# RobotLocomotion/pytorch-dense-correspondence

Measured on AMD Instinct MI355X. Metric: training images/sec, 640x480 D=3 ResNet34-8s, higher is better.
Workload: dtype f32 (f16x3 products)

## Files before the change

include/dcn_hip.h:

```cpp
#ifndef DCN_HIP_H
#define DCN_HIP_H

#include <stddef.h>
#include <stdint.h>

#ifdef __cplusplus
extern "C" {
#endif

#define DCN_OK 0
#define DCN_E_INVALID (-1)
#define DCN_E_LAUNCH (-2)
#define DCN_E_UNSUPPORTED (-3)

const char* dcn_version(void);

void dcn_reload_env(void);

void dcn_release_pooled_buffers(void);


enum { DCN_LIST_MATCH = 0, DCN_LIST_MASKED = 1, DCN_LIST_BACKGROUND = 2, DCN_LIST_BLIND = 3, DCN_NUM_LISTS = 4 };

enum {
// ... 185 lines not shown
size_t dcn_conv_gemm_workspace_hl(const dcn_conv_desc* c, int dgrad);
int dcn_conv_hl_shape_info(const dcn_conv_desc* c, int dgrad, int* info6);
int dcn_split_act_hl32(const float* src, const float* absmax, void* dst, int64_t rows, int channels, void* stream);
int dcn_split_weights_hl32(int n, const float* const* w, void* const* out, const int* cout, const int* taps, const int* cin,
                           const int* ldn, int transposed, float scale, void* stream);
int dcn_conv_forward_hl(const dcn_conv_desc* c, const void* in_hl, const float* in_absmax, const void* w_hl, float w_scale,
                        const float* bias, float* out, float* bn_partial, void* workspace, void* stream);
int dcn_conv_dgrad_hl(const dcn_conv_desc* c, const void* dout_hl, const void* wt_hl, float w_scale, const float* dout_absmax,
                      const float* add, float* din, void* workspace, void* stream);

int dcn_conv_wgrad_hl_eligible(const dcn_conv_desc* c);
int dcn_conv_wgrad_hl_kind(const dcn_conv_desc* c);
size_t dcn_conv_wgrad_workspace_hl(const dcn_conv_desc* c);
int dcn_conv_wgrad_hl(const dcn_conv_desc* c, const void* x_hl, const float* x_absmax, const void* dout_hl,
                      const float* dout_absmax, float* dw, void* slabs, void* stream);

int dcn_split_stem_weights_f16(const float* w4, void* hi, void* lo, int cout, float scale, void* stream);
int dcn_conv_stem_forward_f16(const dcn_conv_desc* c, const float* in, const float* in_absmax, const void* w_hi, const void* w_lo,
                              float w_scale, float* out, float* bn_partial, void* stream);

int dcn_split_weights_f16(int n, const float* const* w, void* const* hi, void* const* lo, const int* cout, const int* taps,
                          const int* cin, const int* ldn, int transposed, float scale, void* stream);

int dcn_split_weights_scaled_f16(int n, const float* const* w, const float* const* row_scale, void* const* hi,
                                 void* const* lo, const int* cout, const int* taps, const int* cin, const int* ldn,
                                 int transposed, float scale, void* stream);
int dcn_conv_forward_fused_f16(const dcn_conv_desc* c, const float* in, const float* in_absmax, const void* w_hi,
                               const void* w_lo, float w_scale, const float* bias, const float* add, int relu, float* out,
                               float* out_absmax, void* workspace, void* stream);

// ... 263 lines not shown
```

pytorch-dense-correspondence_amd/csrc/backbone_engine.hip:

```cpp
#include <algorithm>
#include <cstdio>
#include <cstdlib>
#include <cstring>
#include <mutex>
#include <string>
#include <vector>

#include "dcn_tuning.h"
#include "elementwise_kernels.h"

namespace {

using dcn::ceil_div;

struct ConvL {
    double flops = 0;
    dcn_conv_desc d;
    int w = -1, b = -1;
    int bn = -1;
    size_t x = 0;
    int cin_true = 0;
    size_t wsplit = 0;
    size_t whl = 0;
    bool hl_any = false;
// ... 16 lines not shown
    size_t in = 0, mid[2] = {0, 0}, out = 0;
    int64_t out_rows = 0;
    int out_c = 0, in_c = 0;
    int64_t in_rows = 0;
    int act_in = -1, act_mid[2] = {-1, -1}, act_out = -1;
    int act_down = -1;
    size_t hl_mid[2] = {0, 0}, hl_in = 0;
    bool has_hl_mid[2] = {false, false}, has_hl_in = false;
};
struct ParamInfo {
    std::string name;
    int64_t shape[4];
    int ndim;
};

enum class Kernel : unsigned char { FP32, F16, HL, STEM8 };
struct ConvRoute { Kernel fwd, dgrad, wgrad; };

}

struct dcn_plan {
    std::string arch, prefix;
    int N = 0, H = 0, W = 0, D = 0, Dp = 0, base = 64;
    int groups = 1;
    bool bottleneck = false;
    std::vector<ConvL> convs;
    std::vector<BnL> bns;
    std::vector<BlockL> blocks;
    std::vector<ParamInfo> params;
    std::vector<std::pair<size_t, size_t>> relu_masks;
    int stem = -1, fc = -1;
// ... 34 lines not shown

namespace {

size_t align64(size_t x) { return (x + 63) & ~size_t(63); }

std::vector<ConvRoute> conv_routes(const dcn_plan& p, int conv_mode, bool reserving = false) {
    std::vector<ConvRoute> rt(p.convs.size(), ConvRoute{Kernel::FP32, Kernel::FP32, Kernel::FP32});
    if (conv_mode != DCN_CONV_F16X3) return rt;
    const dcn::Tuning& tune = dcn::tuning();
    for (const ConvL& c : p.convs) {
        ConvRoute& r = rt[c.idx];
        r.fwd = c.hl_any && dcn_conv_hl_eligible(&c.d, 0) != 0 ? Kernel::HL : Kernel::F16;
        r.dgrad = c.hl_any && dcn_conv_hl_eligible(&c.d, 1) != 0 ? Kernel::HL : Kernel::F16;
        const bool hl_x = reserving ? (c.idx != p.stem && c.idx != p.fc) : c.has_hl_x;
        r.wgrad = hl_x && dcn_conv_wgrad_hl_eligible(&c.d) != 0 ? Kernel::HL : Kernel::F16;
    }
    const dcn_conv_desc& sd = p.convs[p.stem].d;
    if (tune.stem8 != 0 && tune.gemm_uni != 0 && sd.win >= 8 && sd.kh == 7 && sd.cin == 4 && (int64_t)sd.n * sd.hin * sd.win * 16 <= ((int64_t)1 << 31))
        rt[p.stem].fwd = Kernel::STEM8;
    return rt;
}

struct Builder {
    dcn_plan& p;
    size_t saved = 0;
    explicit Builder(dcn_plan& pl) : p(pl) {}

    size_t alloc_saved(size_t floats) {
        const size_t o = saved;
        saved = align64(saved + floats);
// ... 910 lines not shown
    auto RT = [&](hipError_t e) { if (e != hipSuccess) rt_fail = 1; };
    if (overlap) {
        hipStreamCaptureStatus cs = hipStreamCaptureStatusNone;
        if (hipStreamIsCapturing(st, &cs) != hipSuccess || cs != hipStreamCaptureStatusNone) overlap = false;
    }
    int n_bn = 0, cur = 0;
    bool wg_pending[2] = {false, false};
    float* const dqbuf[2] = {R.Wk(p.w_dq), R.Wk(p.w_dq2)};
    float* const hlimg[2] = {R.hlbuf(0), R.hlbuf(1)};
    const float* dq_of = nullptr;
    const bool fuse_red = f16 && dcn::tuning().bn_bwd_fused != 0;
    p.fused_bn_bwd = 0;
    const float* red_dy = nullptr;
    int red_tiles = 0;
    const float* hl_dx_of = nullptr;
    auto bn_bwd = [&](const ConvL& c, const float* dy, const float* relu_out, float* dx, float* g_out, const float* dy2 = nullptr) {
        const BnL& b = p.bns[c.bn];
        const float* s = R.S(b.stats);
        const unsigned char* mask = relu_out ? R.M((size_t)(relu_out - R.saved)) : nullptr;
        cur = overlap ? (n_bn & 1) : 0;
        if (overlap && wg_pending[cur]) RT(hipStreamWaitEvent(st, p.ev_wg[cur], 0));
        const int tiles = (red_dy == dy && dy) ? red_tiles : 0;
        red_dy = nullptr;
        if (tiles > 0) { relu_out = nullptr; mask = nullptr; g_out = nullptr; ++p.fused_bn_bwd; }
        const bool prod = f16 && dcn::tuning().hl_producers != 0;
        const bool hl_d = prod && !fuse_red && routes[c.idx].dgrad == Kernel::HL;
        const bool hl_w = prod && routes[c.idx].wgrad == Kernel::HL;
        hl_dx_of = (hl_d || hl_w) ? dx : nullptr;
        dcn::launch_bn_bwd(dy, relu_out, mask, R.S(c.x), s, R.P(b.g), b.C, b.rows, p.groups, part, grads[b.g],
                           grads[b.b], k123, dx, g_out, f16 ? amax + c.idx : nullptr,
                           (f16 && !hl_w) ? (void*)dqbuf[cur] : nullptr, st, tiles, dy2,
                           (hl_d || hl_w) ? (void*)hlimg[cur] : nullptr, hl_d ? 0 : 1,
                           (overlap && dcn::tuning().bn_bwd_lean != 0) ? dcn::tuning().bn_bwd_lean_mask : 0);
        if (overlap) RT(hipEventRecord(p.ev_dq[cur], st));
        ++n_bn;
        dq_of = (f16 && !hl_w) ? dx : nullptr;
    };
    auto wgrad_launch = [&](const ConvL& c, auto&& launch) -> int {
        if (!overlap) return R.timed(1, c.flops, [&] { return launch(st); });
        RT(hipStreamWaitEvent(p.side, p.ev_dq[cur], 0));
        DCN_TRY(launch(p.side));
        RT(hipEventRecord(p.ev_wg[cur], p.side));
        wg_pending[cur] = true;
        return DCN_OK;
    };
    auto wgrad = [&](const ConvL& c, const float* in, const float* dx, float* dw) -> int {
        const Kernel k = routes[c.idx].wgrad;
        if (k == Kernel::FP32) return R.timed(1, c.flops, [&] { return dcn_conv_wgrad(&c.d, in, dx, dw, slab, st); });
        if (k == Kernel::HL) {
            const float* ximg = R.S(c.hl_x);
            if (hl_dx_of != dx) {
                DCN_TRY(R.other([&] { return dcn_split_act_hl32(dx, amax + c.idx, hlimg[cur], (int64_t)c.d.n * c.d.hout * c.d.wout, c.d.ldc, st); }));
                if (overlap) RT(hipEventRecord(p.ev_dq[cur], st));
                hl_dx_of = dx;
            }
            return wgrad_launch(c, [&](hipStream_t s) {
                return dcn_conv_wgrad_hl(&c.d, ximg, R.A(c.in_act), hlimg[cur], amax + c.idx, dw, slab, s);
            });
        }
        if (dq_of != dx) {
            DCN_TRY(R.other([&] { return dcn_split_grad_blocked_f16(dx, c.d.n * c.d.hout * c.d.wout, c.d.ldc, amax + c.idx, dqbuf[0], st); }));
            return R.timed(1, c.flops, [&] {
                return dcn_conv_wgrad_f16(&c.d, in, 1, R.A(c.in_act), dqbuf[0], amax + c.idx, dw, slab, st);
            });
        }
        return wgrad_launch(c, [&](hipStream_t s) {
            return dcn_conv_wgrad_f16(&c.d, in, 1, R.A(c.in_act), dqbuf[cur], amax + c.idx, dw, slab, s);
        });
    };
    auto dgrad = [&](const ConvL& c, const float* dx, const float* add, float* din, const ConvL* bn_of = nullptr,
                     const float* relu_out = nullptr) -> int {
        const ConvRoute& r = routes[c.idx];
        if (r.dgrad == Kernel::FP32) {
            DCN_TRY(R.other([&] { return dcn_transpose_weight(R.P(c.w), wt, c.d.cout, c.d.kh * c.d.kw, c.d.cin, c.d.ldc, st); }));
            return R.timed(0, c.flops, [&] { return dcn_conv_dgrad(&c.d, dx, wt, add, din, R.SK(c, 1, Kernel::FP32), st); });
        }
        if (fuse_red && bn_of) {
            const BnL& b = p.bns[bn_of->bn];
            const int tiles = dcn_conv_dgrad_bn_num_mtiles_f16(&c.d);
            if (tiles > 0 && tiles % p.groups == 0 && b.C == c.d.cin && b.rows == (int64_t)c.d.n * c.d.hin * c.d.win) {
                const unsigned char* mask = relu_out ? R.M((size_t)(relu_out - R.saved)) : nullptr;
                red_dy = din;
                red_tiles = tiles / p.groups;
// ... 107 lines not shown
        float* t = dout; dout = dnext; dnext = t;
        for (size_t k = 0; k + 1 < p.bucket_block.size(); ++k)
            if (p.bucket_block[k] == bi && p.bucket_state == 1) {
                if (overlap) {
                    RT(hipEventRecord(p.ev_bucket_side, p.side));
                    RT(hipStreamWaitEvent(st, p.ev_bucket_side, 0));
                }
                RT(hipEventRecord(p.ev_bucket[k], st));
            }
    }
    const ConvL& stem = p.convs[p.stem];
    const BnL& sb = p.bns[stem.bn];
    const int hp = (stem.d.hout + 2 - 3) / 2 + 1, wp = (stem.d.wout + 2 - 3) / 2 + 1;
    dcn::launch_maxpool_bwd(dout, (const unsigned char*)R.S(p.s_argmax), dnext, N, stem.d.hout, stem.d.wout, hp, wp, sb.C,
                            st, dout_add);
    bn_bwd(stem, dnext, R.S(p.s_stem_y), dxa, nullptr);
    DCN_TRY(wgrad(stem, R.S(p.s_in4), dxa, R.Wk(p.w_dwstem)));
    if (overlap) {
        RT(hipEventRecord(p.ev_join, p.side));
        RT(hipStreamWaitEvent(st, p.ev_join, 0));
    }
    dcn::launch_unpad_c4_to_c3(R.Wk(p.w_dwstem), grads[stem.w], (int64_t)p.base * 49, st);
    if (p.bucket_state == 1) RT(hipEventRecord(p.ev_bucket.back(), st));
    if (rt_fail) return DCN_E_LAUNCH;
    return dcn::check_launch();
}

}

extern "C" int dcn_backbone_backward(dcn_plan* plan, const float* grad_descriptors, const float* const* params,
                                     const void* saved, void* workspace, float* const* grads, int normalize,
// ... 10 lines not shown
```

pytorch-dense-correspondence_amd/csrc/conv_f16_kernels.hip:

```cpp
#include <algorithm>
#include <atomic>

#include "conv_shared.h"
#include "dcn_tuning.h"
#include "f16_split.h"

namespace {

using namespace dcnconv;
using namespace dcnsplit;

constexpr int HBK = 32;
constexpr int LDH = HBK + 8;

__global__ void __launch_bounds__(256)
split_rows_kernel(const float* __restrict__ w, _Float16* __restrict__ hi, _Float16* __restrict__ lo, int64_t rows, int K,
                  int kp, float s) {
    const int64_t i = (int64_t)blockIdx.x * 256 + threadIdx.x;
    const int q = kp / 4;
    if (i >= rows * q) return;
    const int64_t r = i / q;
    const int k = (int)(i - r * q) * 4;
    float4 v = make_float4(0.f, 0.f, 0.f, 0.f);
    if (k < K) v = *reinterpret_cast<const float4*>(w + r * K + k);
// ... 1187 lines not shown
extern "C" size_t dcn_grad_blocked_bytes(int m, int ld) { return (size_t)((m + 3) / 4) * 4 * (size_t)ld * 4; }

extern "C" int dcn_split_grad_blocked_f16(const float* dy, int m, int ld, const float* absmax, void* dq, void* stream) {
    if (!dy || !dq || m < 1 || ld < 4 || (ld % 4) != 0) return DCN_E_INVALID;
    const int64_t total = (int64_t)((m + 3) / 4) * (ld / 4);
    const unsigned blocks = (unsigned)(dcn::ceil_div64(total, 256) > 8192 ? 8192 : dcn::ceil_div64(total, 256));
    hipLaunchKernelGGL(split_grad_blocked_kernel, dim3(blocks), dim3(256), 0, (hipStream_t)stream, dy, m, ld, absmax,
                       (u32x4*)dq);
    return dcn::check_launch();
}

extern "C" size_t dcn_conv_wgrad_workspace_f16(const dcn_conv_desc* c) {
    if (!valid_desc16(c)) return 0;
    int rps;
    const int splits = std::max(wgrad_splits_f16(c, &rps, false), wgrad_splits_f16(c, &rps, c->cout >= 256 && (c->cout % 256) == 0));
    return (size_t)splits * c->cout * c->kh * c->kw * c->cin * sizeof(float);
}

extern "C" int dcn_conv_wgrad_f16(const dcn_conv_desc* c, const void* xs, int xs_is_fp32, const float* x_absmax,
                                  const void* dq, const float* dout_absmax, float* dw, void* slabs, void* stream) {
    if (!valid_desc16(c) || !xs || !dq || !dw || !slabs || (c->ldc % 4) != 0) return DCN_E_INVALID;
    const int64_t x_bytes = (int64_t)c->n * c->hin * c->win * c->cin * 4;
    const int64_t d_bytes = (int64_t)dcn_grad_blocked_bytes(c->n * c->hout * c->wout, c->ldc);
    if (x_bytes > ((int64_t)1 << 31) || d_bytes > ((int64_t)1 << 31)) return DCN_E_UNSUPPORTED;
    WgradF16 p;
    p.xs = xs; p.dq = dq;
    p.d_absmax = dout_absmax; p.x_absmax = xs_is_fp32 ? x_absmax : nullptr; p.x_bytes = (unsigned)x_bytes; p.d_bytes = (unsigned)d_bytes;
    p.hin = c->hin; p.win = c->win; p.cin = c->cin; p.hout = c->hout; p.wout = c->wout; p.cout = c->cout;
    p.kh = c->kh; p.kw = c->kw; p.stride = c->stride; p.pad = c->pad; p.dil = c->dil; p.ldo = c->ldc;
    p.M = c->n * c->hout * c->wout; p.K = c->kh * c->kw * c->cin;
    const bool narrow = c->cout <= 64, wide = wgrad_wide_f16(c);
// ... 37 lines not shown
```

pytorch-dense-correspondence_amd/csrc/conv_shared.h:

```cpp
#pragma once
#include <cstdlib>

#include "dcn_common.h"

namespace dcnconv {

typedef float f32x16 __attribute__((ext_vector_type(16)));

constexpr int NT = 256;

struct FastDiv {
    uint32_t mul, shr;
    int d;
};
inline FastDiv make_fastdiv(int d) {
    FastDiv f;
    f.d = d;
    uint32_t s = 0;
    while ((1u << s) < (uint32_t)d) ++s;
    f.shr = s;
    f.mul = (uint32_t)((((uint64_t)1 << 32) * (((uint64_t)1 << s) - (uint64_t)d)) / (uint64_t)d) + 1u;
    return f;
}
__device__ __forceinline__ int fdiv(int n, const FastDiv& f) { return (int)((__umulhi((uint32_t)n, f.mul) + (uint32_t)n) >> f.shr); }
// ... 237 lines not shown
            }
        }
        __syncthreads();
        if (tid < BN && n0 + tid < p.cd) {
            const float s = red[0 * BN + tid] + red[3 * BN + tid];
            const float q = red[1 * BN + tid] + red[4 * BN + tid];
            const float mx = fmaxf(red[2 * BN + tid], red[5 * BN + tid]);
            p.bn_partial[((int64_t)mt * 3 + 0) * p.cd + n0 + tid] = s;
            p.bn_partial[((int64_t)mt * 3 + 1) * p.cd + n0 + tid] = q;
            p.bn_partial[((int64_t)mt * 3 + 2) * p.cd + n0 + tid] = mx;
        }
    }
}

void launch_wgrad_reduce(const float* slabs, float* dw, int64_t n4, int splits, hipStream_t st);

}
```

pytorch-dense-correspondence_amd/csrc/dcn_tuning.h:

```cpp
#pragma once

namespace dcn {

struct Tuning {
    int conv_mode = -1;
    int conv_mode_invalid = 0;
    int backward_overlap = 1;
    int gemm_tile_m = 0;
    int gemm_sk = -1;
    double gemm_sk_min_gain = 20.0;
    int gemm_uni = 1;
    int stem8 = 1;
    int gemm_sk_inline = 1;
    int bn_bwd_fused = 0;
    int defer_residual_add = 1;
    int wgrad_splits = 0;
    int wgrad_tile = 0;
    int wgrad_deep = 4;
    int gemm_hl = 1;
    int hl_min_k = 128;
    int gemm_hl_rows = 0;
    int gemm_hlx = 1;
    int gemm_hlx_kg = 0;
    int gemm_hlx_splits = 0;
// ... 5 lines not shown
    int wgrad_hl_min_m = 0;
    int wgrad_hl = 1;
    int wgrad_hlr = 1;
    int wgrad_hlr_min_m = 0;
    int wgrad_hlr_pairs = 1;
    int hl_producers = 1;
    int hl_only_mid = 1;
    int stem_pool_fused = 1;
    int bn_reduce_wide = 32;
    int wsplit_overlap = 1;
    int bn_nt = 0;
    int bn_reverse = 0;
    int bn_bwd_lean = 1;
    int bn_bwd_lean_mask = 7;
    int bn_bwd_lean_depth = 3;
    int wgrad_roles = 1;
};

const Tuning& tuning();

}
```

pytorch-dense-correspondence_amd/csrc/dcn_tuning.hip:

```cpp
#include <atomic>
#include <cstdio>
#include <cstdlib>
#include <cstring>
#include <mutex>

#include "dcn_common.h"
#include "dcn_tuning.h"

namespace dcn {
namespace {

Tuning g_tuning;
std::once_flag g_once;
std::mutex g_mu;

void read_env(Tuning& t) {
    t = Tuning();
    if (const char* m = getenv("DCN_CONV_MODE")) {
        if (!strcmp(m, "fp32")) t.conv_mode = DCN_CONV_FP32;
        else if (!strcmp(m, "f16x3")) t.conv_mode = DCN_CONV_F16X3;
        else t.conv_mode_invalid = 1;
    }
    if (const char* e = getenv("DCN_BACKWARD_OVERLAP")) t.backward_overlap = atoi(e) != 0;
    if (const char* e = getenv("DCN_GEMM_TILE_M")) t.gemm_tile_m = atoi(e);
// ... 33 lines not shown
    if (const char* e = getenv("DCN_WGRAD_HL")) t.wgrad_hl = atoi(e);
    if (const char* e = getenv("DCN_HL_SETPRIO")) t.hl_setprio = atoi(e) != 0;
    if (const char* e = getenv("DCN_HLX_STAGGER")) { const int v = atoi(e); t.hlx_stagger = (v >= 0 && v <= 2) ? v : 1; }
    if (const char* e = getenv("DCN_HLX_COUNTERS")) t.hlx_counters = atoi(e) != 0;
    if (const char* e = getenv("DCN_WGRAD_HL_MIN_M")) t.wgrad_hl_min_m = atoi(e);
    if (const char* e = getenv("DCN_WGRAD_HLR")) t.wgrad_hlr = atoi(e);
    if (const char* e = getenv("DCN_WGRAD_HLR_MIN_M")) t.wgrad_hlr_min_m = atoi(e);
    if (const char* e = getenv("DCN_WGRAD_HLR_PAIRS")) t.wgrad_hlr_pairs = atoi(e);
    if (const char* e = getenv("DCN_HL_PRODUCERS")) t.hl_producers = atoi(e) != 0;
    if (const char* e = getenv("DCN_BN_REVERSE")) t.bn_reverse = atoi(e);
    if (const char* e = getenv("DCN_BN_NT")) t.bn_nt = atoi(e);
    if (const char* e = getenv("DCN_WSPLIT_OVERLAP")) t.wsplit_overlap = atoi(e) != 0;
    if (const char* e = getenv("DCN_BN_REDUCE_WIDE")) t.bn_reduce_wide = atoi(e);
    if (const char* e = getenv("DCN_BN_BWD_LEAN")) t.bn_bwd_lean = atoi(e) != 0;
    if (const char* e = getenv("DCN_BN_BWD_LEAN_MASK")) t.bn_bwd_lean_mask = atoi(e) & 7;
    if (const char* e = getenv("DCN_BN_BWD_LEAN_DEPTH")) { const int v = atoi(e); t.bn_bwd_lean_depth = v < 1 ? 1 : (v > 3 ? 3 : v); }
}

}

const Tuning& tuning() {
    std::call_once(g_once, [] { read_env(g_tuning); });
    return g_tuning;
}

}

extern "C" void dcn_reload_env(void) {
    (void)dcn::tuning();
    std::lock_guard<std::mutex> lock(dcn::g_mu);
// ... 3 lines not shown
```

pytorch-dense-correspondence_amd/csrc/elementwise_kernels.hip:

```cpp
#include "dcn_tuning.h"
#include "elementwise_kernels.h"
#include "f16_split.h"

namespace dcn {

__device__ __forceinline__ void wave_atomic_absmax(float amax, float* absmax) {
#pragma unroll
    for (int o = 32; o > 0; o >>= 1) amax = fmaxf(amax, __shfl_xor(amax, o));
    if ((threadIdx.x & 63) == 0 && amax > 0.f) {
        const unsigned bits = __float_as_uint(amax);
        if (bits > __atomic_load_n(reinterpret_cast<unsigned*>(absmax), __ATOMIC_RELAXED))
            atomicMax(reinterpret_cast<unsigned*>(absmax), bits);
    }
}

__global__ void __launch_bounds__(256)
nchw3_to_nhwc4_kernel(const float* __restrict__ img, float* __restrict__ out, int hw, int64_t total,
                      float* __restrict__ absmax) {
    __shared__ float s_m[4];
    float m = 0.f;
    for (int64_t i = (int64_t)blockIdx.x * 256 + threadIdx.x; i < total; i += (int64_t)gridDim.x * 256) {
        const int64_t n = i / hw, p = i - n * hw;
        const float* s = img + n * 3 * hw + p;
        const float4 v = make_float4(s[0], s[hw], s[2 * (int64_t)hw], 0.f);
// ... 1010 lines not shown
        else DCN_BN_RED(K, 16)
        if (lean & 1) { DCN_BN_RED_CQ(bn_bwd_reduce_lean_kernel); }
        else { DCN_BN_RED_CQ(bn_bwd_reduce_kernel); }
#undef DCN_BN_RED_CQ
#undef DCN_BN_RED
    }
    {
        ObservedLaunch obs(DCN_PROF_BN_FINALIZE, 16.0 * (double)chunks * groups * C, st);
        const auto kernel = (lean & 2) ? bn_bwd_finalize_lean_kernel : bn_bwd_finalize_kernel;
        hipLaunchKernelGGL(kernel, dim3(ceil_div(C, 4)), dim3(256), 0, st,
                           (const float*)partial, chunks, groups, C, (double)rpg, gamma, invstd, 4 * C, dgamma, dbeta, k123, absmax);
    }
    const int64_t total4 = rows * (C / 4);
    if ((dq || (hl_dx && (C % 32) == 0)) && absmax) {
        const bool hl = hl_dx && (C % 32) == 0;
        ObservedLaunch obs(DCN_PROF_BN_BWD_APPLY, (double)rows * C * (in_bytes + ((hl && !keep_dx) ? 0.0 : 4.0) + (g_out ? 4.0 : 0.0) +
                                                                      (dq ? 4.0 : 0.0) + (hl ? 4.0 : 0.0)), st);
        const bool deep_apply = deep && C <= 512 && groups <= 2;
        const auto kernel = !(lean & 4) ? bn_bwd_apply_blocked_kernel
                            : (!deep_apply ? (dq ? bn_bwd_apply_blocked_lean_kernel<true> : bn_bwd_apply_blocked_lean_kernel<false>)
                               : (dq ? bn_bwd_apply_blocked_deep_kernel<2, true>
                                     : (depth > 2 ? bn_bwd_apply_blocked_deep_kernel<3, false> : bn_bwd_apply_blocked_deep_kernel<2, false>)));
        hipLaunchKernelGGL(kernel, dim3(blocks_for(((rows + 3) / 4) * (C / 4), kGridCap)), dim3(256), 0, st,
                           dy, dy2, relu_out, relu_mask, x, mean, invstd, (const float*)k123, (const float*)(k123 + C),
                           (const float*)(k123 + 2 * C), (hl_dx && (C % 32) == 0 && !keep_dx) ? nullptr : dx, g_out,
                           (dcnsplit::u32x4*)dq, (const float*)absmax, C / 4, rows, rpg, 4 * C, 3 * C,
                           (C % 32) == 0 ? (dcnsplit::u32x2*)hl_dx : nullptr, (tuning().bn_reverse >> 1) & 1, (tuning().bn_nt >> 1) & 1);
        return;
    }
    ObservedLaunch obs(DCN_PROF_BN_BWD_APPLY, (double)rows * C * (in_bytes + 4.0 + (g_out ? 4.0 : 0.0)), st);
    hipLaunchKernelGGL(bn_bwd_apply_kernel, dim3(blocks_for(total4, kGridCap)), dim3(256), 0, st, dy, dy2, relu_out, relu_mask,
                       x, mean, invstd, (const float*)k123, (const float*)(k123 + C), (const float*)(k123 + 2 * C), dx, g_out,
                       C / 4, total4, total4 / groups, 4 * C, 3 * C, (tuning().bn_reverse >> 1) & 1);
}
void launch_add(const float* a, const float* b, float* out, int64_t n, hipStream_t st) {
    ObservedLaunch obs(DCN_PROF_OTHER, 12.0 * (double)n, st);
    hipLaunchKernelGGL(add_kernel, dim3(blocks_for(n / 4, kGridCap)), dim3(256), 0, st, a, b, out, n / 4);
}
void launch_maxpool_fwd(const float* in, float* out, unsigned char* argmax, int n, int hin, int win, int hout,
                        int wout, int C, hipStream_t st, const float* bn_stats, int groups, unsigned char* relu_mask) {
// ... 119 lines not shown
extern "C" size_t dcn_bn_backward_full_workspace(int64_t rows, int c, int groups) {
    if (rows < 1 || c < 4 || groups < 1 || (rows % groups) != 0) return 0;
    return ((size_t)groups * dcn::bn_bwd_chunks(rows / groups) * 4 * (size_t)c + (size_t)groups * 3 * (size_t)c) * sizeof(float);
}

extern "C" int dcn_bn_backward_full(const float* dy, const float* dy2, const float* relu_out, const unsigned char* relu_mask,
                                    const float* x, const float* stats, const float* gamma, int c, int64_t rows, int groups,
                                    float* dgamma, float* dbeta, float* dx, float* g_out, float* absmax, void* dq, void* hl_dx,
                                    int keep_dx, void* workspace, void* stream) {
    if (!dy || !x || !stats || !gamma || !dgamma || !dbeta || !workspace || c < 4 || (c % 4) != 0 || rows < 1) return DCN_E_INVALID;
    if ((groups != 1 && groups != 2) || (rows % groups) != 0) return DCN_E_INVALID;
    const bool blocked = (dq || (hl_dx && (c % 32) == 0)) && absmax;
    if ((dq || hl_dx) && !absmax) return DCN_E_INVALID;
    if (hl_dx && (c % 32) != 0) return DCN_E_INVALID;
    if (blocked && groups == 2 && ((rows / groups) % 4) != 0) return DCN_E_INVALID;
    if (!dx && !(hl_dx && !keep_dx)) return DCN_E_INVALID;
    float* partial = (float*)workspace;
    float* k123 = partial + (size_t)groups * dcn::bn_bwd_chunks(rows / groups) * 4 * c;
    dcn::launch_bn_bwd(dy, relu_out, relu_mask, x, stats, gamma, c, rows, groups, partial, dgamma, dbeta, k123, dx, g_out, absmax,
                       dq, (hipStream_t)stream, 0, dy2, hl_dx, keep_dx, dcn::tuning().bn_bwd_lean ? dcn::tuning().bn_bwd_lean_mask : 0);
    return dcn::check_launch();
}

extern "C" int dcn_maxpool_forward(const float* in, int n, int hin, int win, int c, float* out, unsigned char* argmax,
                                   void* stream) {
    if (!in || !out || n < 1 || hin < 1 || win < 1 || c < 4 || (c % 4) != 0) return DCN_E_INVALID;
    dcn::launch_maxpool_fwd(in, out, argmax, n, hin, win, (hin + 2 - 3) / 2 + 1, (win + 2 - 3) / 2 + 1, c, (hipStream_t)stream);
    return dcn::check_launch();
}

extern "C" int dcn_maxpool_backward(const float* gout, const unsigned char* argmax, int n, int hin, int win, int c,
// ... 6 lines not shown
```

pytorch-dense-correspondence_amd/dcn_hip/_lib.py:

```python
import atexit
import ctypes
import os

import torch

HERE = os.path.dirname(os.path.abspath(__file__))
DEFAULT_PATH = os.path.join(HERE, "libdcn_hip.so")

_lib = None
_info = {"path": None, "version": None, "hostemu": False}
_reset_hooks = []

c_void_p, c_int, c_int64, c_size_t, c_float, c_char_p = (ctypes.c_void_p, ctypes.c_int, ctypes.c_int64,
                                                         ctypes.c_size_t, ctypes.c_float, ctypes.c_char_p)


class LossConfig(ctypes.Structure):
    _fields_ = [("margin", c_float * 4), ("invert", ctypes.c_int32 * 4), ("pixel_weight", ctypes.c_int32 * 4),
                ("m_pixel", c_float), ("image_width", ctypes.c_int32), ("match_loss_weight", c_float),
                ("non_match_loss_weight", c_float), ("scale_by_hard_negatives", ctypes.c_int32),
                ("compose", ctypes.c_int32)]


class ConvDesc(ctypes.Structure):
# ... 136 lines not shown
                                     c_void_p, c_void_p, c_void_p, c_void_p, c_void_p]),
    "dcn_find_best_match": (c_int, [c_void_p, c_int64, c_int, c_void_p, c_int, c_void_p, c_void_p, c_void_p, c_void_p,
                                    c_void_p, c_void_p]),
    "dcn_find_best_match_workspace": (c_size_t, [c_int]),
    "dcn_upsample_forward": (c_int, [c_void_p, c_int, c_int, c_int, c_int, c_int, c_int, c_int, c_int, c_void_p,
                                     c_void_p]),
    "dcn_upsample_backward": (c_int, [c_void_p, c_int, c_int, c_int, c_int, c_int, c_int, c_int, c_void_p, c_void_p,
                                      c_void_p]),
    "dcn_upsample_backward_tmp_bytes": (c_size_t, [c_int, c_int, c_int, c_int]),
    "dcn_split_weights_checked_f16": (c_int, [c_int, c_void_p, c_void_p, c_void_p, c_void_p, c_void_p, c_void_p, c_void_p,
                                              c_float, c_void_p, c_void_p]),
    "dcn_conv_wgrad_hl_eligible": (c_int, [ctypes.POINTER(ConvDesc)]),
    "dcn_conv_wgrad_hl_kind": (c_int, [ctypes.POINTER(ConvDesc)]),
    "dcn_conv_wgrad_workspace_hl": (c_size_t, [ctypes.POINTER(ConvDesc)]),
    "dcn_conv_wgrad_hl": (c_int, [ctypes.POINTER(ConvDesc), c_void_p, c_void_p, c_void_p, c_void_p, c_void_p, c_void_p, c_void_p]),
    "dcn_conv_hl_eligible": (c_int, [ctypes.POINTER(ConvDesc), c_int]),
    "dcn_conv_num_mtiles_hl": (c_int, [ctypes.POINTER(ConvDesc)]),
    "dcn_conv_tile_rows_hl": (c_int, [ctypes.POINTER(ConvDesc), c_int]),
    "dcn_conv_gemm_workspace_hl": (c_size_t, [ctypes.POINTER(ConvDesc), c_int]),
    "dcn_conv_hl_shape_info": (c_int, [ctypes.POINTER(ConvDesc), c_int, ctypes.POINTER(c_int)]),
    "dcn_split_act_hl32": (c_int, [c_void_p, c_void_p, c_void_p, c_int64, c_int, c_void_p]),
    "dcn_split_weights_hl32": (c_int, [c_int, c_void_p, c_void_p, c_void_p, c_void_p, c_void_p, c_void_p, c_int, c_float,
                                       c_void_p]),
    "dcn_conv_forward_hl": (c_int, [ctypes.POINTER(ConvDesc), c_void_p, c_void_p, c_void_p, c_float, c_void_p, c_void_p,
                                    c_void_p, c_void_p, c_void_p]),
    "dcn_conv_dgrad_hl": (c_int, [ctypes.POINTER(ConvDesc), c_void_p, c_void_p, c_float, c_void_p, c_void_p, c_void_p,
                                  c_void_p, c_void_p]),
    "dcn_augment_images": (c_int, [c_int, c_int, c_int, c_void_p, c_void_p, c_void_p, c_void_p, c_void_p, c_void_p, c_void_p,
                                   c_void_p, c_void_p, c_void_p, c_void_p, c_void_p, c_void_p, c_void_p, c_void_p]),
    "dcn_flip_planes": (c_int, [c_void_p, c_void_p, c_int64, c_int, c_int, c_int, c_int, c_int, c_void_p]),
# ... 120 lines not shown
```

Before: 471.4.

## Add dedicated stem weight-gradient kernel and skip dead stem dx store

Adds a specialised 7x7 stride-2 stem wgrad kernel. It builds input patches in an LDS ring buffer from fp32 input split into f16 hi/lo, and runs three-product MFMA against the blocked f16 gradient image. The kernel sits behind an env flag that defaults off. Separately, the stem's batchnorm backward no longer writes the fp32 dx when only the f16 quantised gradient is consumed, which saves one full-resolution store. The risk is reading a never-written dx if the quantised buffer does not match.

```diff
diff --git a/include/dcn_hip.h b/include/dcn_hip.h
--- a/include/dcn_hip.h
+++ b/include/dcn_hip.h
@@ -223,6 +223,10 @@
 size_t dcn_conv_wgrad_workspace_hl(const dcn_conv_desc* c);
 int dcn_conv_wgrad_hl(const dcn_conv_desc* c, const void* x_hl, const float* x_absmax, const void* dout_hl,
                       const float* dout_absmax, float* dw, void* slabs, void* stream);
+
+int dcn_conv_wgrad_stem_eligible(const dcn_conv_desc* c);
+int dcn_conv_wgrad_stem(const dcn_conv_desc* c, const float* x4, const void* dq_image, const float* dout_absmax, float* dw,
+                        void* slabs, void* stream);
 
 int dcn_split_stem_weights_f16(const float* w4, void* hi, void* lo, int cout, float scale, void* stream);
 int dcn_conv_stem_forward_f16(const dcn_conv_desc* c, const float* in, const float* in_absmax, const void* w_hi, const void* w_lo,
diff --git a/pytorch-dense-correspondence_amd/csrc/backbone_engine.hip b/pytorch-dense-correspondence_amd/csrc/backbone_engine.hip
--- a/pytorch-dense-correspondence_amd/csrc/backbone_engine.hip
+++ b/pytorch-dense-correspondence_amd/csrc/backbone_engine.hip
@@ -54,7 +54,7 @@
     int ndim;
 };
 
-enum class Kernel : unsigned char { FP32, F16, HL, STEM8 };
+enum class Kernel : unsigned char { FP32, F16, HL, STEM8, STEMW };
 struct ConvRoute { Kernel fwd, dgrad, wgrad; };
 
 }
@@ -119,6 +119,7 @@
         r.dgrad = c.hl_any && dcn_conv_hl_eligible(&c.d, 1) != 0 ? Kernel::HL : Kernel::F16;
         const bool hl_x = reserving ? (c.idx != p.stem && c.idx != p.fc) : c.has_hl_x;
         r.wgrad = hl_x && dcn_conv_wgrad_hl_eligible(&c.d) != 0 ? Kernel::HL : Kernel::F16;
+        if (r.wgrad == Kernel::F16 && dcn_conv_wgrad_stem_eligible(&c.d) != 0) r.wgrad = Kernel::STEMW;
     }
     const dcn_conv_desc& sd = p.convs[p.stem].d;
     if (tune.stem8 != 0 && tune.gemm_uni != 0 && sd.win >= 8 && sd.kh == 7 && sd.cin == 4 && (int64_t)sd.n * sd.hin * sd.win * 16 <= ((int64_t)1 << 31))
@@ -1059,7 +1060,8 @@
     const float* red_dy = nullptr;
     int red_tiles = 0;
     const float* hl_dx_of = nullptr;
-    auto bn_bwd = [&](const ConvL& c, const float* dy, const float* relu_out, float* dx, float* g_out, const float* dy2 = nullptr) {
+    auto bn_bwd = [&](const ConvL& c, const float* dy, const float* relu_out, float* dx, float* g_out, const float* dy2 = nullptr,
+                      bool dx_read = true) {
         const BnL& b = p.bns[c.bn];
         const float* s = R.S(b.stats);
         const unsigned char* mask = relu_out ? R.M((size_t)(relu_out - R.saved)) : nullptr;
@@ -1072,8 +1074,10 @@
         const bool hl_d = prod && !fuse_red && routes[c.idx].dgrad == Kernel::HL;
         const bool hl_w = prod && routes[c.idx].wgrad == Kernel::HL;
         hl_dx_of = (hl_d || hl_w) ? dx : nullptr;
+        const bool dx_dead = !dx_read && f16 && !hl_d && !hl_w &&
+                             (routes[c.idx].wgrad == Kernel::F16 || routes[c.idx].wgrad == Kernel::STEMW);
         dcn::launch_bn_bwd(dy, relu_out, mask, R.S(c.x), s, R.P(b.g), b.C, b.rows, p.groups, part, grads[b.g],
-                           grads[b.b], k123, dx, g_out, f16 ? amax + c.idx : nullptr,
+                           grads[b.b], k123, dx_dead ? nullptr : dx, g_out, f16 ? amax + c.idx : nullptr,
                            (f16 && !hl_w) ? (void*)dqbuf[cur] : nullptr, st, tiles, dy2,
                            (hl_d || hl_w) ? (void*)hlimg[cur] : nullptr, hl_d ? 0 : 1,
                            (overlap && dcn::tuning().bn_bwd_lean != 0) ? dcn::tuning().bn_bwd_lean_mask : 0);
@@ -1103,15 +1107,15 @@
                 return dcn_conv_wgrad_hl(&c.d, ximg, R.A(c.in_act), hlimg[cur], amax + c.idx, dw, slab, s);
             });
         }
+        auto launch = [&](const float* dq, hipStream_t s) {
+            if (k == Kernel::STEMW) return dcn_conv_wgrad_stem(&c.d, in, dq, amax + c.idx, dw, slab, s);
+            return dcn_conv_wgrad_f16(&c.d, in, 1, R.A(c.in_act), dq, amax + c.idx, dw, slab, s);
+        };
         if (dq_of != dx) {
             DCN_TRY(R.other([&] { return dcn_split_grad_blocked_f16(dx, c.d.n * c.d.hout * c.d.wout, c.d.ldc, amax + c.idx, dqbuf[0], st); }));
-            return R.timed(1, c.flops, [&] {
-                return dcn_conv_wgrad_f16(&c.d, in, 1, R.A(c.in_act), dqbuf[0], amax + c.idx, dw, slab, st);
-            });
-        }
-        return wgrad_launch(c, [&](hipStream_t s) {
-            return dcn_conv_wgrad_f16(&c.d, in, 1, R.A(c.in_act), dqbuf[cur], amax + c.idx, dw, slab, s);
-        });
+            return R.timed(1, c.flops, [&] { return launch(dqbuf[0], st); });
+        }
+        return wgrad_launch(c, [&](hipStream_t s) { return launch(dqbuf[cur], s); });
     };
     auto dgrad = [&](const ConvL& c, const float* dx, const float* add, float* din, const ConvL* bn_of = nullptr,
                      const float* relu_out = nullptr) -> int {
@@ -1249,7 +1253,7 @@
     const int hp = (stem.d.hout + 2 - 3) / 2 + 1, wp = (stem.d.wout + 2 - 3) / 2 + 1;
     dcn::launch_maxpool_bwd(dout, (const unsigned char*)R.S(p.s_argmax), dnext, N, stem.d.hout, stem.d.wout, hp, wp, sb.C,
                             st, dout_add);
-    bn_bwd(stem, dnext, R.S(p.s_stem_y), dxa, nullptr);
+    bn_bwd(stem, dnext, R.S(p.s_stem_y), dxa, nullptr, nullptr, false);
     DCN_TRY(wgrad(stem, R.S(p.s_in4), dxa, R.Wk(p.w_dwstem)));
     if (overlap) {
         RT(hipEventRecord(p.ev_join, p.side));
diff --git a/pytorch-dense-correspondence_amd/csrc/conv_f16_kernels.hip b/pytorch-dense-correspondence_amd/csrc/conv_f16_kernels.hip
--- a/pytorch-dense-correspondence_amd/csrc/conv_f16_kernels.hip
+++ b/pytorch-dense-correspondence_amd/csrc/conv_f16_kernels.hip
@@ -1225,7 +1225,7 @@
     if (!valid_desc16(c)) return 0;
     int rps;
     const int splits = std::max(wgrad_splits_f16(c, &rps, false), wgrad_splits_f16(c, &rps, c->cout >= 256 && (c->cout % 256) == 0));
-    return (size_t)splits * c->cout * c->kh * c->kw * c->cin * sizeof(float);
+    return std::max((size_t)splits * c->cout * c->kh * c->kw * c->cin * sizeof(float), wgrad_stem_slab_bytes(c));
 }
 
 extern "C" int dcn_conv_wgrad_f16(const dcn_conv_desc* c, const void* xs, int xs_is_fp32, const float* x_absmax,
diff --git a/pytorch-dense-correspondence_amd/csrc/conv_shared.h b/pytorch-dense-correspondence_amd/csrc/conv_shared.h
--- a/pytorch-dense-correspondence_amd/csrc/conv_shared.h
+++ b/pytorch-dense-correspondence_amd/csrc/conv_shared.h
@@ -275,5 +275,6 @@
 }
 
 void launch_wgrad_reduce(const float* slabs, float* dw, int64_t n4, int splits, hipStream_t st);
-
-}
+size_t wgrad_stem_slab_bytes(const dcn_conv_desc* c);
+
+}
diff --git a/pytorch-dense-correspondence_amd/csrc/dcn_tuning.h b/pytorch-dense-correspondence_amd/csrc/dcn_tuning.h
--- a/pytorch-dense-correspondence_amd/csrc/dcn_tuning.h
+++ b/pytorch-dense-correspondence_amd/csrc/dcn_tuning.h
@@ -43,6 +43,7 @@
     int bn_bwd_lean = 1;
     int bn_bwd_lean_mask = 7;
     int bn_bwd_lean_depth = 3;
+    int stem_wgrad = 0;
     int wgrad_roles = 1;
 };
 
diff --git a/pytorch-dense-correspondence_amd/csrc/dcn_tuning.hip b/pytorch-dense-correspondence_amd/csrc/dcn_tuning.hip
--- a/pytorch-dense-correspondence_amd/csrc/dcn_tuning.hip
+++ b/pytorch-dense-correspondence_amd/csrc/dcn_tuning.hip
@@ -71,6 +71,7 @@
     if (const char* e = getenv("DCN_BN_REDUCE_WIDE")) t.bn_reduce_wide = atoi(e);
     if (const char* e = getenv("DCN_BN_BWD_LEAN")) t.bn_bwd_lean = atoi(e) != 0;
     if (const char* e = getenv("DCN_BN_BWD_LEAN_MASK")) t.bn_bwd_lean_mask = atoi(e) & 7;
+    if (const char* e = getenv("DCN_STEM_WGRAD")) t.stem_wgrad = atoi(e) != 0;
     if (const char* e = getenv("DCN_BN_BWD_LEAN_DEPTH")) { const int v = atoi(e); t.bn_bwd_lean_depth = v < 1 ? 1 : (v > 3 ? 3 : v); }
 }
 
diff --git a/pytorch-dense-correspondence_amd/csrc/elementwise_kernels.hip b/pytorch-dense-correspondence_amd/csrc/elementwise_kernels.hip
--- a/pytorch-dense-correspondence_amd/csrc/elementwise_kernels.hip
+++ b/pytorch-dense-correspondence_amd/csrc/elementwise_kernels.hip
@@ -1048,7 +1048,8 @@
     const int64_t total4 = rows * (C / 4);
     if ((dq || (hl_dx && (C % 32) == 0)) && absmax) {
         const bool hl = hl_dx && (C % 32) == 0;
-        ObservedLaunch obs(DCN_PROF_BN_BWD_APPLY, (double)rows * C * (in_bytes + ((hl && !keep_dx) ? 0.0 : 4.0) + (g_out ? 4.0 : 0.0) +
+        float* const dx_st = (hl && !keep_dx) ? nullptr : dx;
+        ObservedLaunch obs(DCN_PROF_BN_BWD_APPLY, (double)rows * C * (in_bytes + (dx_st ? 4.0 : 0.0) + (g_out ? 4.0 : 0.0) +
                                                                       (dq ? 4.0 : 0.0) + (hl ? 4.0 : 0.0)), st);
         const bool deep_apply = deep && C <= 512 && groups <= 2;
         const auto kernel = !(lean & 4) ? bn_bwd_apply_blocked_kernel
@@ -1057,7 +1058,7 @@
                                      : (depth > 2 ? bn_bwd_apply_blocked_deep_kernel<3, false> : bn_bwd_apply_blocked_deep_kernel<2, false>)));
         hipLaunchKernelGGL(kernel, dim3(blocks_for(((rows + 3) / 4) * (C / 4), kGridCap)), dim3(256), 0, st,
                            dy, dy2, relu_out, relu_mask, x, mean, invstd, (const float*)k123, (const float*)(k123 + C),
-                           (const float*)(k123 + 2 * C), (hl_dx && (C % 32) == 0 && !keep_dx) ? nullptr : dx, g_out,
+                           (const float*)(k123 + 2 * C), dx_st, g_out,
                            (dcnsplit::u32x4*)dq, (const float*)absmax, C / 4, rows, rpg, 4 * C, 3 * C,
                            (C % 32) == 0 ? (dcnsplit::u32x2*)hl_dx : nullptr, (tuning().bn_reverse >> 1) & 1, (tuning().bn_nt >> 1) & 1);
         return;
@@ -1207,7 +1208,7 @@
     if ((dq || hl_dx) && !absmax) return DCN_E_INVALID;
     if (hl_dx && (c % 32) != 0) return DCN_E_INVALID;
     if (blocked && groups == 2 && ((rows / groups) % 4) != 0) return DCN_E_INVALID;
-    if (!dx && !(hl_dx && !keep_dx)) return DCN_E_INVALID;
+    if (!dx && !blocked) return DCN_E_INVALID;
     float* partial = (float*)workspace;
     float* k123 = partial + (size_t)groups * dcn::bn_bwd_chunks(rows / groups) * 4 * c;
     dcn::launch_bn_bwd(dy, relu_out, relu_mask, x, stats, gamma, c, rows, groups, partial, dgamma, dbeta, k123, dx, g_out, absmax,
diff --git a/pytorch-dense-correspondence_amd/csrc/wgrad_stem_kernels.hip b/pytorch-dense-correspondence_amd/csrc/wgrad_stem_kernels.hip
--- /dev/null
+++ b/pytorch-dense-correspondence_amd/csrc/wgrad_stem_kernels.hip
@@ -0,0 +1,225 @@
+#include <algorithm>
+
+#include "conv_shared.h"
+#include "dcn_tuning.h"
+#include "f16_split.h"
+
+namespace {
+
+using namespace dcnconv;
+using namespace dcnsplit;
+
+typedef float f32x4 __attribute__((ext_vector_type(4)));
+typedef h8 h8u __attribute__((aligned(2)));
+
+constexpr int kOob = (int)0x80000000;
+constexpr int kHcp = 360;
+constexpr int kMaxChunks = 11;
+constexpr int kRingSlot = 2 * 2 * 4 * kHcp;
+constexpr int kRing = 8 * kRingSlot;
+constexpr int kLda = 40;
+constexpr int kATile = 2 * 64 * kLda;
+constexpr int kK = 196;
+
+struct WgradStem {
+    const float* x;
+    const void* dq;
+    float* slab;
+    const float* d_absmax;
+    unsigned d_bytes;
+    int hin, win, hout, wout, cout, c4n, rows, rows_per_split, ntiles, nch, aligned;
+};
+
+__global__ void __launch_bounds__(512)
+conv_wgrad_stem_kernel(WgradStem p) {
+    __shared__ __attribute__((aligned(16))) _Float16 ring[kRing];
+    __shared__ __attribute__((aligned(16))) _Float16 sa[2 * kATile];
+    const int tid = threadIdx.x, lane = tid & 63;
+    const int wv = __builtin_amdgcn_readfirstlane(tid >> 6);
+    const int mh = wv & 1, nq = wv >> 1;
+    const int fr = lane & 15, fq = lane >> 4;
+    const int split = blockIdx.x / p.ntiles, tile = blockIdx.x - split * p.ntiles;
+    const int g_begin = split * p.rows_per_split;
+    const int g_end = min(p.rows, g_begin + p.rows_per_split);
+    const __amdgpu_buffer_rsrc_t rs_d = __builtin_amdgcn_make_buffer_rsrc(const_cast<void*>(p.dq), 0, (int)p.d_bytes, 0x00020000);
+
+    int brow[4], bconst[4];
+#pragma unroll
+    for (int t = 0; t < 4; ++t) {
+        const int n = 16 * (nq + 4 * t) + fr;
+        const int nv = n < kK ? n : 0;
+        const int tap = nv >> 2, c = nv & 3;
+        const int r = tap / 7, s = tap - 7 * r;
+        brow[t] = r;
+        bconst[t] = (((s + 1) & 1) * 4 + c) * kHcp + ((s + 1) >> 1) + 8 * fq;
+    }
+    const bool tile3 = nq == 0;
+
+    f32x4 acc[2][4];
+#pragma unroll
+    for (int i = 0; i < 2; ++i)
+#pragma unroll
+        for (int t = 0; t < 4; ++t) acc[i][t] = f32x4{0.f, 0.f, 0.f, 0.f};
+
+    const int qq0 = tid >> 6, hl0 = (tid >> 5) & 1, cp0 = tid & 31;
+    const int cg0 = 64 * tile + 2 * cp0;
+    const unsigned sub0 = (unsigned)(hl0 * 2 + (cp0 & 1)) * (unsigned)p.c4n + (unsigned)(cg0 >> 2);
+    const bool second = !p.aligned && tid < 64;
+    u32x4 pa = {0u, 0u, 0u, 0u}, pb = {0u, 0u, 0u, 0u};
+    auto a_issue = [&](int m0, int c0) {
+        const int mf = m0 + c0, qf = mf >> 2, sh = mf & 3;
+        const bool ok0 = c0 + 4 * qq0 - sh < p.wout;
+        pa = __builtin_amdgcn_raw_buffer_load_b128(rs_d, ok0 ? (int)((((unsigned)(qf + qq0) * 4u) * (unsigned)p.c4n + sub0) * 16u) : kOob, 0, 0);
+        if (second) {
+            const bool ok1 = c0 + 32 - sh < p.wout;
+            pb = __builtin_amdgcn_raw_buffer_load_b128(rs_d, ok1 ? (int)((((unsigned)(qf + 8) * 4u) * (unsigned)p.c4n + sub0) * 16u) : kOob, 0, 0);
+        }
+    };
+    auto a_store_piece = [&](_Float16* dst, const u32x4& v, int qq, int sh, int c0) {
+#pragma unroll
+        for (int e = 0; e < 2; ++e)
+#pragma unroll
+            for (int i = 0; i < 4; ++i) {
+                const int j = 4 * qq + i - sh;
+                const unsigned w = v[2 * e + (i >> 1)];
+                const unsigned short bits = (unsigned short)((i & 1) ? (w >> 16) : (w & 0xffffu));
+                if (j >= 0 && j < 32)
+                    reinterpret_cast<unsigned short*>(dst)[e * kLda + j] = (c0 + j < p.wout) ? bits : (unsigned short)0;
+            }
+    };
+    auto a_store = [&](int buf, int m0, int c0) {
+        _Float16* dst = sa + buf * kATile + (hl0 * 64 + 2 * cp0) * kLda;
+        if (p.aligned) {
+            *reinterpret_cast<u32x2*>(dst + 4 * qq0) = u32x2{pa[0], pa[1]};
+            *reinterpret_cast<u32x2*>(dst + kLda + 4 * qq0) = u32x2{pa[2], pa[3]};
+        } else {
+            const int sh = (m0 + c0) & 3;
+            a_store_piece(dst, pa, qq0, sh, c0);
+            if (second) a_store_piece(dst, pb, 8, sh, c0);
+        }
+    };
+    const int used = 32 * p.nch + 8, ucount = 2 * used;
+    auto ring_fill = [&](int img, int ra, int rb) {
+        const int total = (rb - ra + 1) * ucount;
+        for (int e = tid; e < total; e += 512) {
+            const int rr = e / ucount, u = e - rr * ucount;
+            const int iy = ra + rr, ix = u - 4;
+            float4 v = make_float4(0.f, 0.f, 0.f, 0.f);
+            if (iy >= 0 && iy < p.hin && ix >= 0 && ix < p.win)
+                v = *reinterpret_cast<const float4*>(p.x + (((int64_t)img * p.hin + iy) * p.win + ix) * 4);
+            h4 hi, lo;
+            split4_unscaled(v, hi, lo);
+            _Float16* d = ring + ((iy + 8) & 7) * kRingSlot + (u & 1) * 4 * kHcp + (u >> 1);
+#pragma unroll
+            for (int c = 0; c < 4; ++c) {
+                d[c * kHcp] = hi[c];
+                d[8 * kHcp + c * kHcp] = lo[c];
+            }
+        }
+    };
+
+    int have_img = -1, have_oy = 0;
+    int buf = 0;
+    for (int g = g_begin; g < g_end; ++g) {
+        const int img = g / p.hout, oy = g - img * p.hout;
+        const int m0 = g * p.wout;
+        if (img == have_img && oy == have_oy + 1) ring_fill(img, 2 * oy + 2, 2 * oy + 3);
+        else ring_fill(img, 2 * oy - 3, 2 * oy + 3);
+        have_img = img; have_oy = oy;
+        a_issue(m0, 0);
+        a_store(buf, m0, 0);
+        __syncthreads();
+        int boff[4];
+#pragma unroll
+        for (int t = 0; t < 4; ++t) boff[t] = ((2 * oy + brow[t] + 5) & 7) * kRingSlot + bconst[t];
+        for (int ch = 0; ch < p.nch; ++ch) {
+            const int c0 = 32 * ch;
+            const bool more = ch + 1 < p.nch;
+            if (more) a_issue(m0, c0 + 32);
+            const _Float16* a = sa + buf * kATile + (32 * mh + fr) * kLda + 8 * fq;
+            h8 ah[2], al[2];
+#pragma unroll
+            for (int mt = 0; mt < 2; ++mt) {
+                ah[mt] = *reinterpret_cast<const h8*>(a + 16 * mt * kLda);
+                al[mt] = *reinterpret_cast<const h8*>(a + 64 * kLda + 16 * mt * kLda);
+            }
+#pragma unroll
+            for (int t = 0; t < 4; ++t) {
+                if (t == 3 && !tile3) break;
+                const h8 bh = *reinterpret_cast<const h8u*>(ring + boff[t] + c0);
+                const h8 bl = *reinterpret_cast<const h8u*>(ring + boff[t] + 8 * kHcp + c0);
+#pragma unroll
+                for (int mt = 0; mt < 2; ++mt) {
+                    acc[mt][t] = __builtin_amdgcn_mfma_f32_16x16x32_f16(al[mt], bh, acc[mt][t], 0, 0, 0);
+                    acc[mt][t] = __builtin_amdgcn_mfma_f32_16x16x32_f16(ah[mt], bl, acc[mt][t], 0, 0, 0);
+                    acc[mt][t] = __builtin_amdgcn_mfma_f32_16x16x32_f16(ah[mt], bh, acc[mt][t], 0, 0, 0);
+                }
+            }
+            if (more) a_store(buf ^ 1, m0, c0 + 32);
+            __syncthreads();
+            buf ^= 1;
+        }
+    }
+    const float inv = 1.f / (p.d_absmax ? pow2_scale(*p.d_absmax) : 1.f);
+    float* out = p.slab + (int64_t)split * p.cout * kK;
+#pragma unroll
+    for (int t = 0; t < 4; ++t) {
+        const int n = 16 * (nq + 4 * t) + fr;
+        if (n >= kK) continue;
+#pragma unroll
+        for (int mt = 0; mt < 2; ++mt)
+#pragma unroll
+            for (int r = 0; r < 4; ++r) {
+                const int co = 64 * tile + 32 * mh + 16 * mt + 4 * fq + r;
+                out[(int64_t)co * kK + n] = acc[mt][t][r] * inv;
+            }
+    }
+}
+
+bool stem_shape(const dcn_conv_desc* c) {
+    return c && c->n > 0 && c->hin > 0 && c->win > 0 && c->cin == 4 && c->kh == 7 && c->kw == 7 && c->stride == 2 && c->pad == 3 &&
+           c->dil == 1 && c->cout >= 64 && (c->cout % 64) == 0 && c->ldc >= c->cout && (c->ldc % 4) == 0 &&
+           c->hout == (c->hin - 1) / 2 + 1 && c->wout == (c->win - 1) / 2 + 1 && c->wout + 3 <= 32 * kMaxChunks &&
+           (int64_t)c->n * c->hin * c->win * 16 <= ((int64_t)1 << 31) &&
+           (int64_t)((c->n * (int64_t)c->hout * c->wout + 3) / 4) * 16 * c->ldc <= ((int64_t)1 << 31);
+}
+
+int stem_splits(const dcn_conv_desc* c, int* rows_per_split, bool forced) {
+    const int rows = c->n * c->hout, tiles = c->cout / 64;
+    int s = std::max(1, std::min(std::max(256 / tiles, 1), rows));
+    if (forced) { const int v = dcn::tuning().wgrad_splits; if (v >= 1 && v <= rows) s = v; }
+    const int rps = dcn::ceil_div(rows, s);
+    *rows_per_split = rps;
+    return dcn::ceil_div(rows, rps);
+}
+
+}
+
+size_t dcnconv::wgrad_stem_slab_bytes(const dcn_conv_desc* c) {
+    if (!stem_shape(c)) return 0;
+    int rps;
+    const int splits = std::max(stem_splits(c, &rps, true), stem_splits(c, &rps, false));
+    return (size_t)splits * c->cout * kK * sizeof(float);
+}
+
+extern "C" int dcn_conv_wgrad_stem_eligible(const dcn_conv_desc* c) {
+    return (dcn::tuning().stem_wgrad != 0 && stem_shape(c)) ? 1 : 0;
+}
+
+extern "C" int dcn_conv_wgrad_stem(const dcn_conv_desc* c, const float* x4, const void* dq_image, const float* dout_absmax,
+                                   float* dw, void* slabs, void* stream) {
+    if (!c || !x4 || !dq_image || !dw || !slabs) return DCN_E_INVALID;
+    if (!stem_shape(c)) return DCN_E_UNSUPPORTED;
+    WgradStem p;
+    p.x = x4; p.dq = dq_image; p.d_absmax = dout_absmax;
+    p.d_bytes = (unsigned)((int64_t)((c->n * (int64_t)c->hout * c->wout + 3) / 4) * 16 * c->ldc);
+    p.hin = c->hin; p.win = c->win; p.hout = c->hout; p.wout = c->wout; p.cout = c->cout; p.c4n = c->ldc / 4;
+    p.rows = c->n * c->hout; p.ntiles = c->cout / 64; p.nch = dcn::ceil_div(c->wout + 3, 32);
+    p.aligned = (c->wout % 4) == 0 ? 1 : 0;
+    const int splits = stem_splits(c, &p.rows_per_split, true);
+    p.slab = splits == 1 ? dw : (float*)slabs;
+    hipStream_t st = (hipStream_t)stream;
+    hipLaunchKernelGGL(conv_wgrad_stem_kernel, dim3(p.ntiles * splits), dim3(512), 0, st, p);
+    if (splits > 1) launch_wgrad_reduce((const float*)slabs, dw, (int64_t)c->cout * kK / 4, splits, st);
+    return dcn::check_launch();
+}
diff --git a/pytorch-dense-correspondence_amd/dcn_hip/_lib.py b/pytorch-dense-correspondence_amd/dcn_hip/_lib.py
--- a/pytorch-dense-correspondence_amd/dcn_hip/_lib.py
+++ b/pytorch-dense-correspondence_amd/dcn_hip/_lib.py
@@ -174,6 +174,8 @@
     "dcn_conv_wgrad_hl_kind": (c_int, [ctypes.POINTER(ConvDesc)]),
     "dcn_conv_wgrad_workspace_hl": (c_size_t, [ctypes.POINTER(ConvDesc)]),
     "dcn_conv_wgrad_hl": (c_int, [ctypes.POINTER(ConvDesc), c_void_p, c_void_p, c_void_p, c_void_p, c_void_p, c_void_p, c_void_p]),
+    "dcn_conv_wgrad_stem_eligible": (c_int, [ctypes.POINTER(ConvDesc)]),
+    "dcn_conv_wgrad_stem": (c_int, [ctypes.POINTER(ConvDesc), c_void_p, c_void_p, c_void_p, c_void_p, c_void_p, c_void_p]),
     "dcn_conv_hl_eligible": (c_int, [ctypes.POINTER(ConvDesc), c_int]),
     "dcn_conv_num_mtiles_hl": (c_int, [ctypes.POINTER(ConvDesc)]),
     "dcn_conv_tile_rows_hl": (c_int, [ctypes.POINTER(ConvDesc), c_int]),
```

After: 467.5. No clear change (-0.8%).
